# ultralytics/yolov3

Measured on AMD Instinct MI355X. Metric: images/sec (640x640) inference+NMS, higher is better.
Workload: dtype f16; 1 GPU; yolov3 inference 640x640 batch=32/GPU fp16 nc=80 + NMS(conf 0.001, iou 0.6, multi_label, max_det 300) [BASELINE configs[1]]; global_batch=32, parallelism=replicas x1 (no data-path collective)

## Files before the change

yolov3_amd/csrc/api.cpp:

```cpp
#include <atomic>
#include <mutex>
#include <stdarg.h>
#include <stdio.h>
#include <stdlib.h>
#include <string.h>

#include "../../include/yolov3_hip.h"
#include "y3_knobs.h"

static thread_local char g_err[512] = "";

void y3_set_error(const char* fmt, ...) {
    va_list ap;
    va_start(ap, fmt);
    vsnprintf(g_err, sizeof(g_err), fmt, ap);
    va_end(ap);
}

extern "C" const char* y3_last_error(void) { return g_err; }
extern "C" int y3_abi_version(void) { return Y3_ABI_VERSION; }

namespace {
struct Knob {
    const char* name;
    long long def;
};
const Knob kKnobs[] = {
    {"conv", 0}, {"conv_ahead", 3}, {"bn_nt_bytes", 64ll << 20},
    {"wgrad", 0}, {"wgrad_xcd", 2}, {"dgrad_quad", 1}, {"spp_direct", 0}, {"wgrad_strip", 1}, {"conv_strip", 1},
    {"conv_v10", 1}, {"v10_mp", 0}, {"v10_blocks", 0}, {"v10_half", 2}, {"v10_ksplit", 1}, {"v10_slices", 0},
    {"v10_group", 1}, {"tile_xcd", 1}, {"conv_1x1s", 1}, {"wgrad_patch", 1}, {"wgrad_blocks", 512}, {"nms_sort", 1},
    {"decode_tile", 1},
};
constexpr int kCount = (int)(sizeof(kKnobs) / sizeof(kKnobs[0]));
static_assert(kCount == Y3K_COUNT, "kKnobs and y3_knob_id (y3_common.h) list the same knobs in the same order");
std::atomic<long long> g_val[kCount];
std::once_flag g_once;

int knob_index(const char* key) {
    for (int i = 0; i < kCount; ++i)
        if (key && !strcmp(key, kKnobs[i].name)) return i;
    return -1;
}
void load_defaults() {
    for (int i = 0; i < kCount; ++i) g_val[i].store(kKnobs[i].def, std::memory_order_relaxed);
    const char* e = getenv("Y3_TUNE");
    if (!e) return;
    char buf[512];
    strncpy(buf, e, sizeof(buf) - 1);
    buf[sizeof(buf) - 1] = 0;
    for (char* tok = strtok(buf, ",;"); tok; tok = strtok(nullptr, ",;")) {
        char* eq = strchr(tok, '=');
        if (!eq) continue;
        *eq = 0;
        const int i = knob_index(tok);
        if (i >= 0) g_val[i].store(atoll(eq + 1), std::memory_order_relaxed);
        else fprintf(stderr, "libyolov3_hip: Y3_TUNE names an unknown knob '%s'\n", tok);
    }
}
}

long long y3_knob(int id) {
    std::call_once(g_once, load_defaults);
    return (id >= 0 && id < kCount) ? g_val[id].load(std::memory_order_relaxed) : 0;
}

extern "C" int y3_tune_set(const char* key, int64_t value) {
    std::call_once(g_once, load_defaults);
    const int i = knob_index(key);
    if (i < 0) {
        y3_set_error("y3_tune_set: unknown knob '%s'", key ? key : "(null)");
        return -1;
    }
    g_val[i].store((long long)value, std::memory_order_relaxed);
    return 0;
}

extern "C" int64_t y3_tune_get(const char* key) {
    std::call_once(g_once, load_defaults);
    const int i = knob_index(key);
    if (i < 0) {
        y3_set_error("y3_tune_get: unknown knob '%s'", key ? key : "(null)");
        return INT64_MIN;
    }
    return (int64_t)g_val[i].load(std::memory_order_relaxed);
}

extern "C" void y3_tune_reset(void) {
    std::call_once(g_once, load_defaults);
    load_defaults();
}
```

yolov3_amd/csrc/stem.hip:

```cpp
#include "../../include/yolov3_hip.h"
#include "y3_common.h"

#include <hip/hip_runtime.h>
#include <stdint.h>
#include <type_traits>
#include <utility>

namespace {

struct StemArgs {
    const void* x;
    const void* w;
    const float* bias;
    void* y;
    int N, Cin, H, W;
    int ypitch, Cout;
    int act;
    int tiles_w, tiles_h;
    float divisor;
    float* stats;
};

constexpr int TR = 8, TW = 64;
constexpr int PR = TR + 2;
// ... 117 lines not shown
        for (int i = 0; i < NI; ++i) {
            const int pl = i * PPI + rp;
            const frag ov = *(const frag*)(wl + pl * RB + ((ch ^ (pl & (CH - 1))) << 4));
            const int gcol = col0 + j0 + pl;
            if (grow < p.H && gcol < p.W && ch * 8 + 8 <= p.Cout) {
                if (want_stats) {
#pragma unroll
                    for (int q = 0; q < 8; ++q) { const float f = to_f32<T>(ov[q]); st0[q] += f; st1[q] += f * f; }
                }
                *(frag*)(yg + ((long long)(n * p.H + grow) * p.W + gcol) * p.ypitch + ch * 8) = ov;
            }
        }
        __builtin_amdgcn_fence(__ATOMIC_RELEASE, "wavefront");
        __builtin_amdgcn_wave_barrier();
    }
    if (want_stats) {
#pragma unroll
        for (int off = CH; off < 64; off <<= 1)
#pragma unroll
            for (int q = 0; q < 8; ++q) { st0[q] += __shfl_xor(st0[q], off, 64); st1[q] += __shfl_xor(st1[q], off, 64); }
        __syncthreads();
        float* red = (float*)patch;
        if (rp == 0) {
#pragma unroll
            for (int q = 0; q < 8; ++q) { red[(wv * CH + ch) * 16 + 2 * q] = st0[q]; red[(wv * CH + ch) * 16 + 2 * q + 1] = st1[q]; }
        }
        __syncthreads();
        if (tid < CH * 16 && (tid >> 4) * 8 + 8 <= p.Cout) {
            const float v = red[tid] + red[CH * 16 + tid] + red[2 * CH * 16 + tid] + red[3 * CH * 16 + tid];
            p.stats[(long long)blockIdx.x * p.Cout * 2 + tid] = v;
        }
    }
}

struct PairArgs {
    const void* x;
    const void* w0;
    const float* b0;
    const void* w1;
    const float* b1;
    void* y;
    int N, Cin, H, W, Ho, Wo, ypitch, act0, act1, kpad1;
    int tiles_w, tiles_h, n_tiles;
    int xcd;
    float divisor;
#ifdef Y3_TIMELINE
    unsigned long long* tl;
#endif
};
#ifdef Y3_TIMELINE
static unsigned long long* g_pair_tl = nullptr;
#define SP_T(i) do { asm volatile("s_waitcnt lgkmcnt(0)" ::: "memory"); const unsigned long long t_ = __builtin_amdgcn_s_memtime(); asm volatile("s_waitcnt lgkmcnt(0)" ::: "memory"); tsum[i] += t_ - tprev; tprev = t_; } while (0)
#else
#define SP_T(i) do { } while (0)
#endif
constexpr int QR = 4, QW = 32;
constexpr int R0 = 2 * QR + 1, C0 = 2 * QW + 1;
constexpr int XR = R0 + 2, XW = C0 + 3;
constexpr int L0E = C0 / 2 + 1, L0ROW = C0 * 64;

template <typename T, typename S>
__global__ __launch_bounds__(256, 2) void stem_pair_kernel(const PairArgs p) {
    typedef typename Mfma16<T>::frag frag;
    typedef T vec4 __attribute__((ext_vector_type(4)));
    typedef unsigned u32x4 __attribute__((ext_vector_type(4)));
    constexpr int PATCH_BYTES = XR * XW * 8, SLICE_BYTES = 4 * 32 * 64;
    constexpr int SCR = PATCH_BYTES > SLICE_BYTES ? PATCH_BYTES : SLICE_BYTES;
    __shared__ __attribute__((aligned(16))) unsigned char scratch[SCR];
    __shared__ __attribute__((aligned(16))) unsigned char l0buf[R0 * L0ROW];
    __shared__ __attribute__((aligned(16))) unsigned char cw0[32 * 48 * 2];
    __shared__ __attribute__((aligned(16))) float cb0[32], cb1[64];

    const int tid = threadIdx.x, lane = tid & 63;
    const int wv = __builtin_amdgcn_readfirstlane(tid >> 6);
    const int frow = lane & 31, fk = lane >> 5;
    const int wc = wv >> 1, wp = wv & 1;

    for (int i = tid; i < 32 * 48 * 2 / 16; i += 256) ((f32x4*)cw0)[i] = ((const f32x4*)p.w0)[i];
    if (tid < 8) ((f32x4*)cb0)[tid] = ((const f32x4*)p.b0)[tid];
    else if (tid < 24) ((f32x4*)cb1)[tid - 8] = ((const f32x4*)p.b1)[tid - 8];
    frag a1f[18];
#pragma unroll
    for (int t = 0; t < 18; ++t) a1f[t] = *(const frag*)((const T*)p.w1 + (long long)(wc * 32 + frow) * p.kpad1 + t * 16 + fk * 8);

    constexpr int NPX = (XR * XW + 255) / 256;
    int prc[NPX];
#pragma unroll
    for (int j = 0; j < NPX; ++j) {
        const int e = tid + j * 256;
        const int pr = e / XW;
        prc[j] = e < XR * XW ? (pr << 8) | (e - pr * XW) : -1;
    }
    constexpr int NT0 = (R0 * C0 + 31) / 32, NJ0 = (NT0 + 3) / 4;
    int l0rd[NJ0], l0wr[NJ0], l0rc[NJ0];
#pragma unroll
    for (int j = 0; j < NJ0; ++j) {
        int q = (wv + 4 * j) * 32 + frow;
        const bool live = q < R0 * C0;
        if (!live) q = R0 * C0 - 1;
        const int r = q / C0, c = q - r * C0, ci = c >> 1;
        l0rd[j] = (r * XW + c + 2 * fk) * 8;
        l0wr[j] = live ? r * L0ROW + ((c & 1) ? L0E * 64 : 0) + ci * 64 + ((fk ^ ((ci >> 2) & 3)) << 4) : -1;
        l0rc[j] = (r << 8) | c;
    }
    const int hw = p.H * p.W;

    T* __restrict__ yg = (T*)p.y;
    S raw[NPX][4];
    bool rin[NPX];
    auto fetch = [&](int tile) {
        int b = tile;
        const int tw = b % p.tiles_w; b /= p.tiles_w;
        const int th = b % p.tiles_h;
        const int n = b / p.tiles_h;
        const int gh0 = 2 * th * QR - 2, gw0 = 2 * tw * QW - 2;
        const S* __restrict__ xs = (const S*)p.x + (long long)n * p.Cin * hw;
#pragma unroll
        for (int j = 0; j < NPX; ++j) {
            const int gh = gh0 + (prc[j] >> 8), gw = gw0 + (prc[j] & 255);
            rin[j] = prc[j] >= 0 && (unsigned)gh < (unsigned)p.H && (unsigned)gw < (unsigned)p.W;
            if (rin[j]) {
                const unsigned o = (unsigned)(gh * p.W + gw);
#pragma unroll
                for (int c = 0; c < 4; ++c)
                    if (c < p.Cin) raw[j][c] = xs[o + (unsigned)(c * hw)];
            }
        }
    };
    const bool plain = std::is_same<S, T>::value && p.divisor == 1.0f;
    auto stash = [&]() {
#pragma unroll
        for (int j = 0; j < NPX; ++j) {
            const int e = tid + j * 256;
            if (e < XR * XW) {
                vec4 v = {(T)0.0f, (T)0.0f, (T)0.0f, (T)0.0f};
                if (rin[j]) {
                    bool done = false;
                    if constexpr (std::is_same<S, T>::value) {
                        if (plain) {
#pragma unroll
                            for (int c = 0; c < 4; ++c)
                                if (c < p.Cin) v[c] = raw[j][c];
                            done = true;
                        }
                    }
                    if (!done) {
#pragma unroll
                        for (int c = 0; c < 4; ++c)
                            if (c < p.Cin) v[c] = from_f32<T>(src_f32<S>(raw[j][c]) / p.divisor);
                    }
                }
                *(vec4*)(scratch + e * 8) = v;
            }
        }
    };
    const int first = p.xcd ? xcd_remap((int)blockIdx.x, (int)gridDim.x) : (int)blockIdx.x;
    if (first < p.n_tiles) fetch(first);
#ifdef Y3_TIMELINE
    unsigned long long tsum[8] = {0, 0, 0, 0, 0, 0, 0, 0};
    unsigned long long tprev = __builtin_amdgcn_s_memtime();
#endif
    for (int tile = first; tile < p.n_tiles; tile += gridDim.x) {
        int b = tile;
        const int tw = b % p.tiles_w; b /= p.tiles_w;
        const int th = b % p.tiles_h;
        const int n = b / p.tiles_h;
        const int oh0 = th * QR, ow0 = tw * QW;
        const int gh0 = 2 * oh0 - 1, gw0 = 2 * ow0 - 1;
        const bool border = gh0 < 0 || gw0 < 0 || gh0 + R0 > p.H || gw0 + C0 > p.W;

        stash();
        SP_T(0);
        __syncthreads();
        SP_T(1);

#pragma unroll
        for (int j = 0; j < NJ0; ++j) {
            if (wv + 4 * j >= NT0) break;
            f32x16 acc;
#pragma unroll
            for (int g = 0; g < 4; ++g)
#pragma unroll
                for (int e = 0; e < 4; ++e) acc[4 * g + e] = cb0[8 * g + 4 * fk + e];
#pragma unroll
            for (int kh = 0; kh < 3; ++kh) {
                const unsigned char* src = scratch + l0rd[j] + kh * (XW * 8);
                typedef unsigned long long u64x2 __attribute__((ext_vector_type(2)));
                u64x2 rw;
                rw[0] = *(const unsigned long long*)src;
                rw[1] = *(const unsigned long long*)(src + 8);
                acc = Mfma16<T>::run(*(const frag*)(cw0 + ((frow * 3 + kh) * 16 + fk * 8) * 2), __builtin_bit_cast(frag, rw), acc);
            }
            if (p.act0 == Y3_ACT_SILU) silu_vec<f32x16, 16>(acc);
            bool keep = l0wr[j] >= 0;
            bool inside = true;
            if (border) inside = (unsigned)(gh0 + (l0rc[j] >> 8)) < (unsigned)p.H && (unsigned)(gw0 + (l0rc[j] & 255)) < (unsigned)p.W;
#pragma unroll
            for (int gp = 0; gp < 2; ++gp) {
                u32x4 ov;
#pragma unroll
                for (int h = 0; h < 2; ++h) {
                    const unsigned a = pack2<T>(acc[8 * gp + 2 * h], acc[8 * gp + 2 * h + 1]);
                    const unsigned b = pack2<T>(acc[8 * gp + 4 + 2 * h], acc[8 * gp + 4 + 2 * h + 1]);
                    const auto sw = __builtin_amdgcn_permlane32_swap(a, b, false, false);
                    ov[h] = inside ? (unsigned)sw[0] : 0u;
                    ov[2 + h] = inside ? (unsigned)sw[1] : 0u;
                }
                if (keep) *(u32x4*)(l0buf + (l0wr[j] ^ (gp << 5))) = ov;
            }
        }
        SP_T(2);
        __syncthreads();
        SP_T(3);
        if (tile + (int)gridDim.x < p.n_tiles) fetch(tile + gridDim.x);

        f32x16 acc1[2];
#pragma unroll
        for (int b2 = 0; b2 < 2; ++b2)
#pragma unroll
            for (int g = 0; g < 4; ++g)
#pragma unroll
                for (int e = 0; e < 4; ++e) acc1[b2][4 * g + e] = cb1[wc * 32 + 8 * g + 4 * fk + e];
#pragma unroll
        for (int tap = 0; tap < 9; ++tap) {
            const int kh = tap / 3, kw = tap - 3 * (tap / 3);
#pragma unroll
            for (int ks = 0; ks < 2; ++ks)
#pragma unroll
                for (int b2 = 0; b2 < 2; ++b2) {
                    const int lr = 2 * wp + b2;
                    const int ci = frow + (kw >> 1);
                    const frag bf = *(const frag*)(l0buf + (2 * lr + kh) * L0ROW + ((kw & 1) ? L0E * 64 : 0) + ci * 64 + (((ks * 2 + fk) ^ ((ci >> 2) & 3)) << 4));
                    acc1[b2] = Mfma16<T>::run(a1f[tap * 2 + ks], bf, acc1[b2]);
                }
        }
        SP_T(4);
        unsigned char* wl = scratch + wv * (32 * 64);
        const int rp = lane >> 2, ch = lane & 3;
        if (p.act1 == Y3_ACT_SILU) {
            silu_vec<f32x16, 16>(acc1[0]);
            silu_vec<f32x16, 16>(acc1[1]);
        }
        const long long ybase = ((long long)(n * p.Ho + oh0 + 2 * wp) * p.Wo + ow0) * p.ypitch + wc * 32 + ch * 8;
#pragma unroll
        for (int b2 = 0; b2 < 2; ++b2) {
#pragma unroll
            for (int gp = 0; gp < 2; ++gp) {
                u32x4 ov;
#pragma unroll
                for (int h = 0; h < 2; ++h) {
                    const unsigned a = pack2<T>(acc1[b2][8 * gp + 2 * h], acc1[b2][8 * gp + 2 * h + 1]);
                    const unsigned b = pack2<T>(acc1[b2][8 * gp + 4 + 2 * h], acc1[b2][8 * gp + 4 + 2 * h + 1]);
                    const auto sw = __builtin_amdgcn_permlane32_swap(a, b, false, false);
                    ov[h] = (unsigned)sw[0];
                    ov[2 + h] = (unsigned)sw[1];
                }
                const int chunk = gp * 2 + fk;
                *(u32x4*)(wl + frow * 64 + ((chunk ^ (frow & 3)) << 4)) = ov;
            }
            __builtin_amdgcn_fence(__ATOMIC_RELEASE, "wavefront");
            __builtin_amdgcn_wave_barrier();
            __builtin_amdgcn_fence(__ATOMIC_ACQUIRE, "wavefront");
            const int oh = oh0 + 2 * wp + b2;
#pragma unroll
            for (int i = 0; i < 2; ++i) {
                const int pl = i * 16 + rp;
                const u32x4 ov = *(const u32x4*)(wl + pl * 64 + ((ch ^ (pl & 3)) << 4));
                if (oh < p.Ho && ow0 + pl < p.Wo) *(u32x4*)(yg + ybase + (long long)(b2 * p.Wo + pl) * p.ypitch) = ov;
            }
            __builtin_amdgcn_fence(__ATOMIC_RELEASE, "wavefront");
            __builtin_amdgcn_wave_barrier();
        }
        SP_T(5);
        __syncthreads();
        SP_T(6);
    }
#ifdef Y3_TIMELINE
    if (p.tl && blockIdx.x < 64 && lane == 0) {
#pragma unroll
        for (int i = 0; i < 8; ++i) p.tl[(blockIdx.x * 4 + wv) * 8 + i] = tsum[i];
    }
#endif
}

struct BneckArgs {
    const void* x;
    const void* w1;
    const float* b1;
    const void* w2;
    const float* b2;
    void* y;
    int N, H, W, xpitch, ypitch, act1, act2, add, kpad1, kpad2;
    int tiles_w, tiles_h, n_tiles;
    int xcd;
    unsigned x_bytes;
};
constexpr int BC = 32, RC = BC + 2;
constexpr int bneck_rows(int c) { return c == 64 ? 8 : 4; }
constexpr int L1PITCH = 40;

template <typename F, int... Is> Y3_DEV void sfor_impl(F&& f, std::integer_sequence<int, Is...>) { (f(std::integral_constant<int, Is>{}), ...); }
template <int N, typename F> Y3_DEV void sfor(F&& f) { sfor_impl(f, std::make_integer_sequence<int, N>{}); }

template <typename T, int C>
__global__ __launch_bounds__(C * 4, C == 64 ? 2 : 1) void bneck_pair_kernel(const BneckArgs p) {
    typedef typename Mfma16<T>::frag frag;
    typedef unsigned u32x4 __attribute__((ext_vector_type(4)));
    typedef __attribute__((address_space(3))) void* lds_ptr_t;
    constexpr int BR = bneck_rows(C), RW = BR / 2;
    constexpr int RR = BR + 2, RPX = RR * RC;
    constexpr int NT1 = (RPX + 31) / 32;
    constexpr int CM = C / 2;
    constexpr int FT = C / 32;
    constexpr int NWV = 2 * FT;
    constexpr int XB = C * 2, XCHK = XB / 16;
    constexpr int LB = CM * 2, LCHK = LB / 16;
    constexpr int K1S = C / 16, M1 = CM / 32;
    constexpr int KT = CM / 16;
    constexpr int K2S = 9 * KT;
    constexpr int XPIECES = (RPX * XCHK + 63) / 64;
    constexpr int XJ = (XPIECES + NWV - 1) / NWV;
    constexpr int NJ1 = (NT1 + NWV - 1) / NWV;
    constexpr int QSTEP = 32 * NWV;
    constexpr int XKS = XCHK == 8 ? 1 : 0;
    constexpr int LKS = LCHK == 4 ? 2 : 1;
    __shared__ __attribute__((aligned(16))) unsigned char xbuf[XPIECES * 1024];
    __shared__ __attribute__((aligned(16))) unsigned char l1buf[RR * L1PITCH * LB];
    __shared__ __attribute__((aligned(16))) unsigned char slices[NWV * 32 * 64];
    __shared__ __attribute__((aligned(16))) float cb1[CM], cb2[C];
    constexpr bool W1_LDS = C == 128;
    __shared__ __attribute__((aligned(16))) unsigned char cw1[W1_LDS ? CM * C * 2 : 16];

    const int tid = threadIdx.x, lane = tid & 63;
    const int wv = __builtin_amdgcn_readfirstlane(tid >> 6);
    const int frow = lane & 31, fk = lane >> 5;
    const int wc = wv >> 1, wp = wv & 1;

    if (tid < CM / 4) ((f32x4*)cb1)[tid] = ((const f32x4*)p.b1)[tid];
    else if (tid < CM / 4 + C / 4) ((f32x4*)cb2)[tid - CM / 4] = ((const f32x4*)p.b2)[tid - CM / 4];
    if constexpr (W1_LDS) {
        for (int i = tid; i < CM * XCHK; i += 64 * NWV) {
            const int r = i / XCHK, c = i % XCHK;
            *(u32x4*)(cw1 + r * XB + ((c ^ (r & 15)) << 4)) = *(const u32x4*)((const T*)p.w1 + (long long)r * p.kpad1 + c * 8);
        }
    }
    frag a2f[K2S];
#pragma unroll
    for (int t = 0; t < K2S; ++t) a2f[t] = *(const frag*)((const T*)p.w2 + (long long)(wc * 32 + frow) * p.kpad2 + t * 16 + fk * 8);

    const auto rs_x = __builtin_amdgcn_make_buffer_rsrc((void*)p.x, 0, (int)p.x_bytes, 0x00020000);
    const int c1q0 = 32 * wv + frow;
    const int c1r0 = c1q0 / RC, c1c0 = c1q0 - c1r0 * RC;
    const int c1rd0 = c1q0 * XB + ((fk ^ ((c1q0 >> XKS) & (XCHK - 1))) << 4);
    int c2rd[3];
#pragma unroll
    for (int kw = 0; kw < 3; ++kw) c2rd[kw] = (frow + kw) * LB + ((fk ^ (((frow + kw) >> LKS) & (LCHK - 1))) << 4);

    T* __restrict__ yg = (T*)p.y;
    auto fetch = [&](int tile) {
        int b = tile;
        const int tw = b % p.tiles_w; b /= p.tiles_w;
        const int th = b % p.tiles_h;
        const int n = b / p.tiles_h;
        const int gh0 = th * BR - 1, gw0 = tw * BC - 1;
        int lane_f = lane;
        asm volatile("" : "+v"(lane_f));
        const int xq0 = (64 / XCHK) * wv + lane_f / XCHK;
        const unsigned xsrc = (unsigned)(((lane_f % XCHK) ^ ((xq0 >> XKS) & (XCHK - 1))) * 16);
        int r = 0, c = xq0;
#pragma unroll
        for (int j = 0; j < XJ; ++j) {
            if (wv + NWV * j >= XPIECES) break;
            const int gh = gh0 + r, gw = gw0 + c;
            const bool ok = xq0 + 32 * j < RPX && (unsigned)gh < (unsigned)p.H && (unsigned)gw < (unsigned)p.W;
            const unsigned off = ok ? (unsigned)(((n * p.H + gh) * p.W + gw) * p.xpitch) * 2u + xsrc : 0xffffffffu;
            const unsigned ldsa = __builtin_amdgcn_readfirstlane((unsigned)(uintptr_t)(lds_ptr_t)xbuf + (unsigned)((wv + NWV * j) * 1024));
            asm volatile("s_mov_b32 m0, %0\n\ts_nop 0\n\tbuffer_load_dwordx4 %1, %2, 0 offen lds" : : "s"(ldsa), "v"(off), "s"(rs_x) : "memory");
            c += 32;
            if (c >= RC) { c -= RC; r += 1; }
        }
    };
    const int first = p.xcd ? xcd_remap((int)blockIdx.x, (int)gridDim.x) : (int)blockIdx.x;
    if (first < p.n_tiles) fetch(first);
    for (int tile = first; tile < p.n_tiles; tile += gridDim.x) {
        int b = tile;
        const int tw = b % p.tiles_w; b /= p.tiles_w;
        const int th = b % p.tiles_h;
        const int n = b / p.tiles_h;
        const int oh0 = th * BR, ow0 = tw * BC;
        const int gh0 = oh0 - 1, gw0 = ow0 - 1;
        const bool border = gh0 < 0 || gw0 < 0 || gh0 + RR > p.H || gw0 + RC > p.W;

        frag a1g[W1_LDS ? 1 : K1S * M1];
        if constexpr (!W1_LDS) {
#pragma unroll
            for (int ks = 0; ks < K1S; ++ks)
#pragma unroll
                for (int m = 0; m < M1; ++m) a1g[ks * M1 + m] = *(const frag*)((const T*)p.w1 + (long long)(m * 32 + frow) * p.kpad1 + ks * 16 + fk * 8);
        }
        __builtin_amdgcn_s_waitcnt(0x0F70);
        __syncthreads();

        {
            f32x16 acc[NJ1][M1];
#pragma unroll
            for (int j = 0; j < NJ1; ++j)
#pragma unroll
                for (int m = 0; m < M1; ++m)
#pragma unroll
                    for (int g = 0; g < 4; ++g)
#pragma unroll
                        for (int e = 0; e < 4; ++e) acc[j][m][4 * g + e] = cb1[m * 32 + 8 * g + 4 * fk + e];
#pragma unroll
            for (int ks = 0; ks < K1S; ++ks) {
                frag af[M1];
#pragma unroll
                for (int m = 0; m < M1; ++m) {
                    if constexpr (W1_LDS) af[m] = *(const frag*)(cw1 + (m * 32 + frow) * XB + (((2 * ks + fk) ^ (frow & 15)) << 4));
                    else af[m] = a1g[ks * M1 + m];
                }
#pragma unroll
                for (int j = 0; j < NJ1; ++j) {
                    if (wv + NWV * j >= NT1) break;
                    const frag bf = *(const frag*)(xbuf + ((c1rd0 + j * (QSTEP * XB)) ^ (ks << 5)));
#pragma unroll
                    for (int m = 0; m < M1; ++m) acc[j][m] = Mfma16<T>::run(af[m], bf, acc[j][m]);
                }
            }
            int r1 = c1r0, c1 = c1c0;
#pragma unroll
            for (int j = 0; j < NJ1; ++j) {
                if (wv + NWV * j >= NT1) break;
                const bool live = c1q0 + QSTEP * j < RPX;
                bool inside = true;
                if (border) inside = (unsigned)(gh0 + r1) < (unsigned)p.H && (unsigned)(gw0 + c1) < (unsigned)p.W;
                const int wr = (r1 * L1PITCH + c1) * LB + ((fk ^ ((c1 >> LKS) & (LCHK - 1)) ^ ((r1 & 1) * (LCHK / 2))) << 4);
#pragma unroll
                for (int m = 0; m < M1; ++m) {
                    if (p.act1 == Y3_ACT_SILU) silu_vec<f32x16, 16>(acc[j][m]);
#pragma unroll
                    for (int gp = 0; gp < 2; ++gp) {
                        u32x4 ov;
#pragma unroll
                        for (int h = 0; h < 2; ++h) {
                            const auto sw = __builtin_amdgcn_permlane32_swap(pack2<T>(acc[j][m][8 * gp + 2 * h], acc[j][m][8 * gp + 2 * h + 1]),
                                                                             pack2<T>(acc[j][m][8 * gp + 4 + 2 * h], acc[j][m][8 * gp + 4 + 2 * h + 1]), false, false);
                            ov[h] = inside ? (unsigned)sw[0] : 0u;
                            ov[2 + h] = inside ? (unsigned)sw[1] : 0u;
                        }
                        if (live) *(u32x4*)(l1buf + (wr ^ ((m * 4 + gp * 2) << 4))) = ov;
                    }
                    __builtin_amdgcn_sched_barrier(0);
                }
                c1 += QSTEP % RC;
                r1 += QSTEP / RC;
                if (c1 >= RC) { c1 -= RC; r1 += 1; }
            }
        }
        u32x4 xres[2 * RW];
        if (p.add) {
            int lane_r = lane;
            asm volatile("" : "+v"(lane_r));
            const int rp_r = lane_r >> 2, lc = wc * 4 + (lane_r & 3);
#pragma unroll
            for (int b2 = 0; b2 < RW; ++b2)
#pragma unroll
                for (int i = 0; i < 2; ++i) {
                    const int q = (RW * wp + b2 + 1) * RC + (i * 16 + rp_r + 1);
                    xres[b2 * 2 + i] = *(const u32x4*)(xbuf + q * XB + ((lc ^ ((q >> XKS) & (XCHK - 1))) << 4));
                }
        }
        __syncthreads();
        {
            int nt = tile + (int)gridDim.x;
            asm volatile("" : "+s"(nt));
            if (nt < p.n_tiles) fetch(nt);
        }
        f32x16 acc2[RW];
#pragma unroll
        for (int b2 = 0; b2 < RW; ++b2)
#pragma unroll
            for (int g = 0; g < 4; ++g)
#pragma unroll
                for (int e = 0; e < 4; ++e) acc2[b2][4 * g + e] = cb2[wc * 32 + 8 * g + 4 * fk + e];
        const unsigned char* l1w = l1buf + (RW * wp) * (L1PITCH * LB);
        auto rd = [&](auto step_c, frag (&bf)[RW]) {
            constexpr int tap = decltype(step_c)::value / KT, ks = decltype(step_c)::value % KT, kh = tap / 3, kw = tap - 3 * (tap / 3);
#pragma unroll
            for (int b2 = 0; b2 < RW; ++b2) {
                const int rr = b2 + kh;
                bf[b2] = *(const frag*)(l1w + rr * (L1PITCH * LB) + (c2rd[kw] ^ (((2 * ks) ^ ((rr & 1) * (LCHK / 2))) << 4)));
            }
        };
        auto mm = [&](auto step_c, const frag (&bf)[RW]) {
#pragma unroll
            for (int b2 = 0; b2 < RW; ++b2) acc2[b2] = Mfma16<T>::run(a2f[decltype(step_c)::value], bf[b2], acc2[b2]);
        };
        frag bA[RW], bB[RW];
        rd(std::integral_constant<int, 0>{}, bA);
        __builtin_amdgcn_sched_barrier(0);
        sfor<K2S / 2 - 1>([&](auto i_c) {
            constexpr int s0 = 2 * decltype(i_c)::value;
            rd(std::integral_constant<int, s0 + 1>{}, bB);
            mm(std::integral_constant<int, s0>{}, bA);
            __builtin_amdgcn_sched_barrier(0);
            rd(std::integral_constant<int, s0 + 2>{}, bA);
            mm(std::integral_constant<int, s0 + 1>{}, bB);
            __builtin_amdgcn_sched_barrier(0);
        });
        rd(std::integral_constant<int, K2S - 1>{}, bB);
        mm(std::integral_constant<int, K2S - 2>{}, bA);
        __builtin_amdgcn_sched_barrier(0);
        mm(std::integral_constant<int, K2S - 1>{}, bB);
        __builtin_amdgcn_sched_barrier(0);
        int lane_o = lane;
        asm volatile("" : "+v"(lane_o));
        const int rp = lane_o >> 2, ch = lane_o & 3;
        unsigned char* wl = slices + wv * (32 * 64);
        if (p.act2 == Y3_ACT_SILU) {
#pragma unroll
            for (int b2 = 0; b2 < RW; ++b2) {
                silu_vec<f32x16, 16>(acc2[b2]);
                __builtin_amdgcn_sched_barrier(0);
            }
        }
        const long long ybase = ((long long)(n * p.H + oh0 + RW * wp) * p.W + ow0) * p.ypitch + wc * 32 + ch * 8;
#pragma unroll
        for (int b2 = 0; b2 < RW; ++b2) {
#pragma unroll
            for (int gp = 0; gp < 2; ++gp) {
                u32x4 ov;
#pragma unroll
                for (int h = 0; h < 2; ++h) {
                    const auto sw = __builtin_amdgcn_permlane32_swap(pack2<T>(acc2[b2][8 * gp + 2 * h], acc2[b2][8 * gp + 2 * h + 1]),
                                                                     pack2<T>(acc2[b2][8 * gp + 4 + 2 * h], acc2[b2][8 * gp + 4 + 2 * h + 1]), false, false);
                    ov[h] = (unsigned)sw[0];
                    ov[2 + h] = (unsigned)sw[1];
                }
                const int chunk = gp * 2 + fk;
                *(u32x4*)(wl + frow * 64 + ((chunk ^ (frow & 3)) << 4)) = ov;
            }
            __builtin_amdgcn_fence(__ATOMIC_RELEASE, "wavefront");
            __builtin_amdgcn_wave_barrier();
            __builtin_amdgcn_fence(__ATOMIC_ACQUIRE, "wavefront");
            const int orow = RW * wp + b2;
#pragma unroll
            for (int i = 0; i < 2; ++i) {
                const int pl = i * 16 + rp;
                frag ov = *(const frag*)(wl + pl * 64 + ((ch ^ (pl & 3)) << 4));
                if (p.add) {
                    const frag xr = __builtin_bit_cast(frag, xres[b2 * 2 + i]);
                    u32x4 sum;
#pragma unroll
                    for (int e = 0; e < 8; e += 2) sum[e >> 1] = pack2<T>(to_f32<T>(ov[e]) + to_f32<T>(xr[e]), to_f32<T>(ov[e + 1]) + to_f32<T>(xr[e + 1]));
                    ov = __builtin_bit_cast(frag, sum);
                }
                if (oh0 + orow < p.H && ow0 + pl < p.W) *(frag*)(yg + ybase + (long long)(b2 * p.W + pl) * p.ypitch) = ov;
            }
            __builtin_amdgcn_fence(__ATOMIC_RELEASE, "wavefront");
            __builtin_amdgcn_wave_barrier();
        }
        __syncthreads();
    }
}

template <typename T, typename S> int launch_stem(const StemArgs& a, hipStream_t st) {
    const dim3 grid((unsigned)((long long)a.tiles_w * a.tiles_h * a.N));
    if (a.Cout <= 32)
        hipLaunchKernelGGL((stem_conv_kernel<T, S, 1>), grid, dim3(256), 0, st, a);
    else
        hipLaunchKernelGGL((stem_conv_kernel<T, S, 2>), grid, dim3(256), 0, st, a);
    Y3_CHECK_LAUNCH();
    return 0;
}

template <typename T> int dispatch_src(const StemArgs& a, int sdt, hipStream_t st) {
    switch (sdt) {
        case Y3_F16: return launch_stem<T, f16_t>(a, st);
        case Y3_BF16: return launch_stem<T, bf16_t>(a, st);
        case Y3_F32: return launch_stem<T, float>(a, st);
        case Y3_U8: return launch_stem<T, unsigned char>(a, st);
    }
    Y3_FAIL("y3_stem_conv_fwd: bad source dtype %d", sdt);
}

}

static int stem_conv_impl(const void* x_nchw, int32_t src_dtype, int32_t n, int32_t cin, int32_t h, int32_t w, float divisor, const void* packed, const float* bias,
                          int32_t dtype, int32_t act, const y3_tensor* y, float* stat_rows, int64_t capacity_rows, int64_t* n_rows, void* stream, const char* who) {
    if (!x_nchw || !packed || !y || !y->data) Y3_FAIL("%s: null argument", who);
    if (cin < 1 || cin > 4) Y3_FAIL("%s: %d input channels (1..4 supported)", who, cin);
    if (y->n != n || y->h != h || y->w != w) Y3_FAIL("%s: output must be (%d,%d,%d,*) for a stride-1 pad-1 3x3", who, n, h, w);
    if ((y->c % 8) || y->c > 64 || (y->pitch % 8) || ((uintptr_t)y->data & 15) || ((uintptr_t)packed & 15)) Y3_FAIL("%s: 8..64 filters (multiple of 8), 16-byte aligned views", who);
    if (!(divisor > 0.0f)) Y3_FAIL("%s: divisor must be positive", who);
    if ((long long)n * h * w > 0x7fffffffLL) Y3_FAIL("%s: too many pixels", who);
    StemArgs a;
    a.x = x_nchw; a.w = packed; a.bias = bias; a.y = y->data;
    a.N = n; a.Cin = cin; a.H = h; a.W = w; a.ypitch = y->pitch; a.Cout = y->c; a.act = act;
    a.tiles_w = (w + TW - 1) / TW; a.tiles_h = (h + TR - 1) / TR;
    a.divisor = divisor;
    a.stats = stat_rows;
    const long long rows = (long long)a.tiles_w * a.tiles_h * n;
    if (stat_rows) {
        if (rows > capacity_rows) Y3_FAIL("%s: %lld statistics rows, capacity %lld", who, rows, (long long)capacity_rows);
        if (n_rows) *n_rows = rows;
    }
    hipStream_t st = (hipStream_t)stream;
    switch (dtype) {
        case Y3_F16: return dispatch_src<f16_t>(a, src_dtype, st);
        case Y3_BF16: return dispatch_src<bf16_t>(a, src_dtype, st);
    }
    Y3_FAIL("%s: f16/bf16 compute only", who);
}

extern "C" int y3_stem_conv_fwd(const void* x_nchw, int32_t src_dtype, int32_t n, int32_t cin, int32_t h, int32_t w, float divisor, const void* packed,
                                const float* bias, int32_t dtype, int32_t act, const y3_tensor* y, void* stream) {
    return stem_conv_impl(x_nchw, src_dtype, n, cin, h, w, divisor, packed, bias, dtype, act, y, nullptr, 0, nullptr, stream, "y3_stem_conv_fwd");
}

extern "C" int64_t y3_stem_conv_stats_rows(int32_t n, int32_t h, int32_t w) { return (int64_t)((w + TW - 1) / TW) * ((h + TR - 1) / TR) * n; }

extern "C" int y3_stem_conv_fwd_stats(const void* x_nchw, int32_t src_dtype, int32_t n, int32_t cin, int32_t h, int32_t w, float divisor, const void* packed,
                                      const float* bias, int32_t dtype, int32_t act, const y3_tensor* y, float* stat_rows, int64_t capacity_rows, int64_t* n_rows,
                                      void* stream) {
    if (!stat_rows || !n_rows) Y3_FAIL("y3_stem_conv_fwd_stats: null statistics buffer");
    return stem_conv_impl(x_nchw, src_dtype, n, cin, h, w, divisor, packed, bias, dtype, act, y, stat_rows, capacity_rows, n_rows, stream, "y3_stem_conv_fwd_stats");
}

namespace {
template <typename T> int dispatch_pair(const PairArgs& a, int sdt, long long tiles, hipStream_t st) {
    const int cap = 2 * y3_cu_count();
    const int blocks = tiles < cap ? (int)tiles : cap;
    switch (sdt) {
        case Y3_F16: hipLaunchKernelGGL((stem_pair_kernel<T, f16_t>), dim3((unsigned)blocks), dim3(256), 0, st, a); break;
        case Y3_BF16: hipLaunchKernelGGL((stem_pair_kernel<T, bf16_t>), dim3((unsigned)blocks), dim3(256), 0, st, a); break;
        case Y3_F32: hipLaunchKernelGGL((stem_pair_kernel<T, float>), dim3((unsigned)blocks), dim3(256), 0, st, a); break;
        case Y3_U8: hipLaunchKernelGGL((stem_pair_kernel<T, unsigned char>), dim3((unsigned)blocks), dim3(256), 0, st, a); break;
        default: Y3_FAIL("y3_stem_pair_fwd: bad source dtype %d", sdt);
    }
    Y3_CHECK_LAUNCH();
    return 0;
}
}

#ifdef Y3_TIMELINE
extern "C" void y3_debug_pair_timeline(void* buf) { g_pair_tl = (unsigned long long*)buf; }
#endif

extern "C" int y3_stem_pair_fwd(const void* x_nchw, int32_t src_dtype, int32_t n, int32_t cin, int32_t h, int32_t w, float divisor, const void* packed0, const float* bias0,
                                int32_t act0, const void* packed1, const float* bias1, int32_t act1, int32_t dtype, const y3_tensor* y, void* stream) {
    if (!x_nchw || !packed0 || !bias0 || !packed1 || !bias1 || !y || !y->data) Y3_FAIL("y3_stem_pair_fwd: null argument");
    if (cin < 1 || cin > 4) Y3_FAIL("y3_stem_pair_fwd: %d input channels (1..4 supported)", cin);
    const int Ho = (h - 1) / 2 + 1, Wo = (w - 1) / 2 + 1;
    if (y->n != n || y->h != Ho || y->w != Wo || y->c != 64) Y3_FAIL("y3_stem_pair_fwd: output must be (%d,%d,%d,64)", n, Ho, Wo);
    if ((y->pitch % 8) || ((uintptr_t)y->data & 15) || ((uintptr_t)packed0 & 15) || ((uintptr_t)packed1 & 15) || ((uintptr_t)bias0 & 15) || ((uintptr_t)bias1 & 15))
        Y3_FAIL("y3_stem_pair_fwd: 16-byte aligned views");
    if (!(divisor > 0.0f)) Y3_FAIL("y3_stem_pair_fwd: divisor must be positive");
    if ((long long)n * h * w > 0x7fffffffLL) Y3_FAIL("y3_stem_pair_fwd: too many pixels");
    PairArgs a;
    a.x = x_nchw; a.w0 = packed0; a.b0 = bias0; a.w1 = packed1; a.b1 = bias1; a.y = y->data;
    a.N = n; a.Cin = cin; a.H = h; a.W = w; a.Ho = Ho; a.Wo = Wo; a.ypitch = y->pitch; a.act0 = act0; a.act1 = act1;
    a.kpad1 = y3_filter_kpad(32, 3);
    a.tiles_w = (Wo + QW - 1) / QW; a.tiles_h = (Ho + QR - 1) / QR;
    const long long tiles = (long long)a.tiles_w * a.tiles_h * n;
    if (tiles > 0x7fffffffLL) Y3_FAIL("y3_stem_pair_fwd: too many tiles");
    a.n_tiles = (int)tiles;
    a.xcd = y3_knob(Y3K_TILE_XCD) != 0;
    a.divisor = divisor;
#ifdef Y3_TIMELINE
    a.tl = g_pair_tl;
#endif
    hipStream_t st = (hipStream_t)stream;
    switch (dtype) {
        case Y3_F16: return dispatch_pair<f16_t>(a, src_dtype, tiles, st);
        case Y3_BF16: return dispatch_pair<bf16_t>(a, src_dtype, tiles, st);
    }
    Y3_FAIL("y3_stem_pair_fwd: f16/bf16 compute only");
}

extern "C" int y3_bneck_pair_fwd(const y3_tensor* x, const void* packed1, const float* bias1, int32_t act1, const void* packed2, const float* bias2, int32_t act2,
                                 int32_t add_residual, int32_t dtype, const y3_tensor* y, void* stream) {
    if (!x || !x->data || !packed1 || !bias1 || !packed2 || !bias2 || !y || !y->data) Y3_FAIL("y3_bneck_pair_fwd: null argument");
    const int c = x->c;
    if ((c != 64 && c != 128) || y->c != c) Y3_FAIL("y3_bneck_pair_fwd: Bottleneck(64, 64) or Bottleneck(128, 128) (cv1 C -> C/2 1x1, cv2 C/2 -> C 3x3), got %d -> %d channels", x->c, y->c);
    if (y->n != x->n || y->h != x->h || y->w != x->w) Y3_FAIL("y3_bneck_pair_fwd: output shape");
    if ((x->pitch % 8) || (y->pitch % 8) || ((uintptr_t)x->data & 15) || ((uintptr_t)y->data & 15) || ((uintptr_t)packed1 & 15) || ((uintptr_t)packed2 & 15) ||
        ((uintptr_t)bias1 & 15) || ((uintptr_t)bias2 & 15))
        Y3_FAIL("y3_bneck_pair_fwd: 16-byte aligned views");
    if (x->data == y->data) Y3_FAIL("y3_bneck_pair_fwd: in-place operation is not supported (tiles read their neighbours' input)");
    BneckArgs a;
    a.x = x->data; a.w1 = packed1; a.b1 = bias1; a.w2 = packed2; a.b2 = bias2; a.y = y->data;
    a.N = x->n; a.H = x->h; a.W = x->w; a.xpitch = x->pitch; a.ypitch = y->pitch; a.act1 = act1; a.act2 = act2; a.add = add_residual ? 1 : 0;
    a.kpad1 = y3_filter_kpad(c, 1); a.kpad2 = y3_filter_kpad(c / 2, 3);
    a.tiles_w = (x->w + BC - 1) / BC; a.tiles_h = (x->h + bneck_rows(c) - 1) / bneck_rows(c);
    const long long tiles = (long long)a.tiles_w * a.tiles_h * x->n;
    if (tiles > 0x7fffffffLL || (long long)x->n * x->h * x->w > 0x7fffffffLL) Y3_FAIL("y3_bneck_pair_fwd: too many pixels");
    a.n_tiles = (int)tiles;
    a.xcd = y3_knob(Y3K_TILE_XCD) != 0;
    const long long xb = (((long long)x->n * x->h * x->w - 1) * x->pitch + x->c) * 2;
    if (xb >= 0x7fffffffLL) Y3_FAIL("y3_bneck_pair_fwd: input beyond the 2 GiB reach of a buffer descriptor (split the batch)");
    a.x_bytes = (unsigned)xb;
    const int cap = (c == 64 ? 2 : 1) * y3_cu_count();
    const int blocks = tiles < cap ? (int)tiles : cap;
    hipStream_t st = (hipStream_t)stream;
    if (dtype != Y3_F16 && dtype != Y3_BF16) Y3_FAIL("y3_bneck_pair_fwd: f16/bf16 only");
    if (c == 64) {
        if (dtype == Y3_F16) hipLaunchKernelGGL((bneck_pair_kernel<f16_t, 64>), dim3((unsigned)blocks), dim3(256), 0, st, a);
        else hipLaunchKernelGGL((bneck_pair_kernel<bf16_t, 64>), dim3((unsigned)blocks), dim3(256), 0, st, a);
    } else {
        if (dtype == Y3_F16) hipLaunchKernelGGL((bneck_pair_kernel<f16_t, 128>), dim3((unsigned)blocks), dim3(512), 0, st, a);
        else hipLaunchKernelGGL((bneck_pair_kernel<bf16_t, 128>), dim3((unsigned)blocks), dim3(512), 0, st, a);
    }
    Y3_CHECK_LAUNCH();
    return 0;
}
```

yolov3_amd/csrc/y3_knobs.h:

```cpp
#pragma once
enum y3_knob_id {
    Y3K_CONV = 0,
    Y3K_CONV_AHEAD,
    Y3K_BN_NT_BYTES,
    Y3K_WGRAD,
    Y3K_WGRAD_XCD,
    Y3K_DGRAD_QUAD,
    Y3K_SPP_DIRECT,
    Y3K_WGRAD_STRIP,
    Y3K_CONV_STRIP,
    Y3K_CONV_V10,
    Y3K_V10_MP,
    Y3K_V10_BLOCKS,
    Y3K_V10_HALF,
    Y3K_V10_KSPLIT,
    Y3K_V10_SLICES,
    Y3K_V10_GROUP,
    Y3K_TILE_XCD,
    Y3K_CONV_1X1S,
    Y3K_WGRAD_PATCH,
    Y3K_WGRAD_BLOCKS,
    Y3K_NMS_SORT,
    Y3K_DECODE_TILE,
    Y3K_COUNT
};
long long y3_knob(int id);
```

Before: 5235 images/sec.

## Pipeline bottleneck-pair epilogue into next row's MFMAs and hoist w1 fragment loads

Adds a PIPE variant of the fused bottleneck-pair kernel, selected by a new pair_pipe knob that is on by default. The variant interleaves each output row's SiLU, permlane packing, LDS transpose and global store into the MFMA stream of the following row, using a three-deep B-fragment rotation. It also loads the 1x1 weight fragments once per block instead of once per tile. The aim is to hide epilogue latency and cut repeated global weight loads, at the cost of more register pressure and a fragile, hand-placed schedule.

```diff
diff --git a/yolov3_amd/csrc/api.cpp b/yolov3_amd/csrc/api.cpp
--- a/yolov3_amd/csrc/api.cpp
+++ b/yolov3_amd/csrc/api.cpp
@@ -30,7 +30,7 @@
     {"wgrad", 0}, {"wgrad_xcd", 2}, {"dgrad_quad", 1}, {"spp_direct", 0}, {"wgrad_strip", 1}, {"conv_strip", 1},
     {"conv_v10", 1}, {"v10_mp", 0}, {"v10_blocks", 0}, {"v10_half", 2}, {"v10_ksplit", 1}, {"v10_slices", 0},
     {"v10_group", 1}, {"tile_xcd", 1}, {"conv_1x1s", 1}, {"wgrad_patch", 1}, {"wgrad_blocks", 512}, {"nms_sort", 1},
-    {"decode_tile", 1},
+    {"decode_tile", 1}, {"pair_pipe", 1},
 };
 constexpr int kCount = (int)(sizeof(kKnobs) / sizeof(kKnobs[0]));
 static_assert(kCount == Y3K_COUNT, "kKnobs and y3_knob_id (y3_common.h) list the same knobs in the same order");
diff --git a/yolov3_amd/csrc/stem.hip b/yolov3_amd/csrc/stem.hip
--- a/yolov3_amd/csrc/stem.hip
+++ b/yolov3_amd/csrc/stem.hip
@@ -443,7 +443,7 @@
 template <typename F, int... Is> Y3_DEV void sfor_impl(F&& f, std::integer_sequence<int, Is...>) { (f(std::integral_constant<int, Is>{}), ...); }
 template <int N, typename F> Y3_DEV void sfor(F&& f) { sfor_impl(f, std::make_integer_sequence<int, N>{}); }
 
-template <typename T, int C>
+template <typename T, int C, int PIPE>
 __global__ __launch_bounds__(C * 4, C == 64 ? 2 : 1) void bneck_pair_kernel(const BneckArgs p) {
     typedef typename Mfma16<T>::frag frag;
     typedef unsigned u32x4 __attribute__((ext_vector_type(4)));
@@ -490,9 +490,6 @@
     for (int t = 0; t < K2S; ++t) a2f[t] = *(const frag*)((const T*)p.w2 + (long long)(wc * 32 + frow) * p.kpad2 + t * 16 + fk * 8);
 
     const auto rs_x = __builtin_amdgcn_make_buffer_rsrc((void*)p.x, 0, (int)p.x_bytes, 0x00020000);
-    const int c1q0 = 32 * wv + frow;
-    const int c1r0 = c1q0 / RC, c1c0 = c1q0 - c1r0 * RC;
-    const int c1rd0 = c1q0 * XB + ((fk ^ ((c1q0 >> XKS) & (XCHK - 1))) << 4);
     int c2rd[3];
 #pragma unroll
     for (int kw = 0; kw < 3; ++kw) c2rd[kw] = (frow + kw) * LB + ((fk ^ (((frow + kw) >> LKS) & (LCHK - 1))) << 4);
@@ -523,6 +520,19 @@
     };
     const int first = p.xcd ? xcd_remap((int)blockIdx.x, (int)gridDim.x) : (int)blockIdx.x;
     if (first < p.n_tiles) fetch(first);
+    frag a1g[W1_LDS ? 1 : K1S * M1];
+    auto load_a1g = [&]() {
+        if constexpr (!W1_LDS) {
+#pragma unroll
+            for (int ks = 0; ks < K1S; ++ks)
+#pragma unroll
+                for (int m = 0; m < M1; ++m) a1g[ks * M1 + m] = *(const frag*)((const T*)p.w1 + (long long)(m * 32 + frow) * p.kpad1 + ks * 16 + fk * 8);
+        }
+    };
+    if constexpr (PIPE) {
+        load_a1g();
+        __builtin_amdgcn_s_waitcnt(0x0F70);
+    }
     for (int tile = first; tile < p.n_tiles; tile += gridDim.x) {
         int b = tile;
         const int tw = b % p.tiles_w; b /= p.tiles_w;
@@ -532,14 +542,13 @@
         const int gh0 = oh0 - 1, gw0 = ow0 - 1;
         const bool border = gh0 < 0 || gw0 < 0 || gh0 + RR > p.H || gw0 + RC > p.W;
 
-        frag a1g[W1_LDS ? 1 : K1S * M1];
-        if constexpr (!W1_LDS) {
-#pragma unroll
-            for (int ks = 0; ks < K1S; ++ks)
-#pragma unroll
-                for (int m = 0; m < M1; ++m) a1g[ks * M1 + m] = *(const frag*)((const T*)p.w1 + (long long)(m * 32 + frow) * p.kpad1 + ks * 16 + fk * 8);
-        }
-        __builtin_amdgcn_s_waitcnt(0x0F70);
+        int lane_c = lane;
+        if constexpr (PIPE) asm volatile("" : "+v"(lane_c));
+        const int c1q0 = 32 * wv + (lane_c & 31);
+        const int c1r0 = c1q0 / RC, c1c0 = c1q0 - c1r0 * RC;
+        const int c1rd0 = c1q0 * XB + (((lane_c >> 5) ^ ((c1q0 >> XKS) & (XCHK - 1))) << 4);
+        if constexpr (!PIPE) load_a1g();
+        if constexpr (!PIPE) __builtin_amdgcn_s_waitcnt(0x0F70);
         __syncthreads();
 
         {
@@ -625,81 +634,169 @@
 #pragma unroll
                 for (int e = 0; e < 4; ++e) acc2[b2][4 * g + e] = cb2[wc * 32 + 8 * g + 4 * fk + e];
         const unsigned char* l1w = l1buf + (RW * wp) * (L1PITCH * LB);
-        auto rd = [&](auto step_c, frag (&bf)[RW]) {
-            constexpr int tap = decltype(step_c)::value / KT, ks = decltype(step_c)::value % KT, kh = tap / 3, kw = tap - 3 * (tap / 3);
+        if constexpr (!PIPE) {
+            auto rd = [&](auto step_c, frag (&bf)[RW]) {
+                constexpr int tap = decltype(step_c)::value / KT, ks = decltype(step_c)::value % KT, kh = tap / 3, kw = tap - 3 * (tap / 3);
+#pragma unroll
+                for (int b2 = 0; b2 < RW; ++b2) {
+                    const int rr = b2 + kh;
+                    bf[b2] = *(const frag*)(l1w + rr * (L1PITCH * LB) + (c2rd[kw] ^ (((2 * ks) ^ ((rr & 1) * (LCHK / 2))) << 4)));
+                }
+            };
+            auto mm = [&](auto step_c, const frag (&bf)[RW]) {
+#pragma unroll
+                for (int b2 = 0; b2 < RW; ++b2) acc2[b2] = Mfma16<T>::run(a2f[decltype(step_c)::value], bf[b2], acc2[b2]);
+            };
+            frag bA[RW], bB[RW];
+            rd(std::integral_constant<int, 0>{}, bA);
+            __builtin_amdgcn_sched_barrier(0);
+            sfor<K2S / 2 - 1>([&](auto i_c) {
+                constexpr int s0 = 2 * decltype(i_c)::value;
+                rd(std::integral_constant<int, s0 + 1>{}, bB);
+                mm(std::integral_constant<int, s0>{}, bA);
+                __builtin_amdgcn_sched_barrier(0);
+                rd(std::integral_constant<int, s0 + 2>{}, bA);
+                mm(std::integral_constant<int, s0 + 1>{}, bB);
+                __builtin_amdgcn_sched_barrier(0);
+            });
+            rd(std::integral_constant<int, K2S - 1>{}, bB);
+            mm(std::integral_constant<int, K2S - 2>{}, bA);
+            __builtin_amdgcn_sched_barrier(0);
+            mm(std::integral_constant<int, K2S - 1>{}, bB);
+            __builtin_amdgcn_sched_barrier(0);
+            int lane_o = lane;
+            asm volatile("" : "+v"(lane_o));
+            const int rp = lane_o >> 2, ch = lane_o & 3;
+            unsigned char* wl = slices + wv * (32 * 64);
+            if (p.act2 == Y3_ACT_SILU) {
+#pragma unroll
+                for (int b2 = 0; b2 < RW; ++b2) {
+                    silu_vec<f32x16, 16>(acc2[b2]);
+                    __builtin_amdgcn_sched_barrier(0);
+                }
+            }
+            const long long ybase = ((long long)(n * p.H + oh0 + RW * wp) * p.W + ow0) * p.ypitch + wc * 32 + ch * 8;
 #pragma unroll
             for (int b2 = 0; b2 < RW; ++b2) {
-                const int rr = b2 + kh;
-                bf[b2] = *(const frag*)(l1w + rr * (L1PITCH * LB) + (c2rd[kw] ^ (((2 * ks) ^ ((rr & 1) * (LCHK / 2))) << 4)));
-            }
-        };
-        auto mm = [&](auto step_c, const frag (&bf)[RW]) {
-#pragma unroll
-            for (int b2 = 0; b2 < RW; ++b2) acc2[b2] = Mfma16<T>::run(a2f[decltype(step_c)::value], bf[b2], acc2[b2]);
-        };
-        frag bA[RW], bB[RW];
-        rd(std::integral_constant<int, 0>{}, bA);
-        __builtin_amdgcn_sched_barrier(0);
-        sfor<K2S / 2 - 1>([&](auto i_c) {
-            constexpr int s0 = 2 * decltype(i_c)::value;
-            rd(std::integral_constant<int, s0 + 1>{}, bB);
-            mm(std::integral_constant<int, s0>{}, bA);
-            __builtin_amdgcn_sched_barrier(0);
-            rd(std::integral_constant<int, s0 + 2>{}, bA);
-            mm(std::integral_constant<int, s0 + 1>{}, bB);
-            __builtin_amdgcn_sched_barrier(0);
-        });
-        rd(std::integral_constant<int, K2S - 1>{}, bB);
-        mm(std::integral_constant<int, K2S - 2>{}, bA);
-        __builtin_amdgcn_sched_barrier(0);
-        mm(std::integral_constant<int, K2S - 1>{}, bB);
-        __builtin_amdgcn_sched_barrier(0);
-        int lane_o = lane;
-        asm volatile("" : "+v"(lane_o));
-        const int rp = lane_o >> 2, ch = lane_o & 3;
-        unsigned char* wl = slices + wv * (32 * 64);
-        if (p.act2 == Y3_ACT_SILU) {
-#pragma unroll
-            for (int b2 = 0; b2 < RW; ++b2) {
-                silu_vec<f32x16, 16>(acc2[b2]);
+#pragma unroll
+                for (int gp = 0; gp < 2; ++gp) {
+                    u32x4 ov;
+#pragma unroll
+                    for (int h = 0; h < 2; ++h) {
+                        const auto sw = __builtin_amdgcn_permlane32_swap(pack2<T>(acc2[b2][8 * gp + 2 * h], acc2[b2][8 * gp + 2 * h + 1]),
+                                                                         pack2<T>(acc2[b2][8 * gp + 4 + 2 * h], acc2[b2][8 * gp + 4 + 2 * h + 1]), false, false);
+                        ov[h] = (unsigned)sw[0];
+                        ov[2 + h] = (unsigned)sw[1];
+                    }
+                    const int chunk = gp * 2 + fk;
+                    *(u32x4*)(wl + frow * 64 + ((chunk ^ (frow & 3)) << 4)) = ov;
+                }
+                __builtin_amdgcn_fence(__ATOMIC_RELEASE, "wavefront");
+                __builtin_amdgcn_wave_barrier();
+                __builtin_amdgcn_fence(__ATOMIC_ACQUIRE, "wavefront");
+                const int orow = RW * wp + b2;
+#pragma unroll
+                for (int i = 0; i < 2; ++i) {
+                    const int pl = i * 16 + rp;
+                    frag ov = *(const frag*)(wl + pl * 64 + ((ch ^ (pl & 3)) << 4));
+                    if (p.add) {
+                        const frag xr = __builtin_bit_cast(frag, xres[b2 * 2 + i]);
+                        u32x4 sum;
+#pragma unroll
+                        for (int e = 0; e < 8; e += 2) sum[e >> 1] = pack2<T>(to_f32<T>(ov[e]) + to_f32<T>(xr[e]), to_f32<T>(ov[e + 1]) + to_f32<T>(xr[e + 1]));
+                        ov = __builtin_bit_cast(frag, sum);
+                    }
+                    if (oh0 + orow < p.H && ow0 + pl < p.W) *(frag*)(yg + ybase + (long long)(b2 * p.W + pl) * p.ypitch) = ov;
+                }
+                __builtin_amdgcn_fence(__ATOMIC_RELEASE, "wavefront");
+                __builtin_amdgcn_wave_barrier();
+            }
+        } else {
+            constexpr int QS = K2S >= 36 ? 5 : 2;
+            constexpr int SW0 = QS + (QS > 2 ? 2 : 1), SW1 = 3 * QS + (QS > 2 ? 2 : 1);
+            constexpr int SRD = 3 * QS + (QS > 2 ? 5 : 3), SST = SRD + 3, SEND = SRD + 7;
+            static_assert(SW0 > QS && SW1 > 3 * QS && SRD > SW1 && SEND < K2S, "the epilogue of a row fits into the MFMAs of the next");
+            const long long ybase = ((long long)(n * p.H + oh0 + RW * wp) * p.W + ow0) * p.ypitch + wc * 32;
+            unsigned char* wl = slices + wv * (32 * 64);
+            frag so[2];
+            auto epi = [&](auto row_c, auto s_c, auto silu_c) {
+                constexpr int b2 = decltype(row_c)::value, s = decltype(s_c)::value;
+                if constexpr (decltype(silu_c)::value && s % QS == 0 && s / QS < 4) {
+                    constexpr int q = 4 * (s / QS);
+                    f32x4 v = {acc2[b2][q], acc2[b2][q + 1], acc2[b2][q + 2], acc2[b2][q + 3]};
+                    silu_vec<f32x4, 4>(v);
+#pragma unroll
+                    for (int e = 0; e < 4; ++e) acc2[b2][q + e] = v[e];
+                }
+                if constexpr (s == SW0 || s == SW1) {
+                    constexpr int gp = s == SW1 ? 1 : 0;
+                    u32x4 ov;
+#pragma unroll
+                    for (int h = 0; h < 2; ++h) {
+                        const auto sw = __builtin_amdgcn_permlane32_swap(pack2<T>(acc2[b2][8 * gp + 2 * h], acc2[b2][8 * gp + 2 * h + 1]),
+                                                                         pack2<T>(acc2[b2][8 * gp + 4 + 2 * h], acc2[b2][8 * gp + 4 + 2 * h + 1]), false, false);
+                        ov[h] = (unsigned)sw[0];
+                        ov[2 + h] = (unsigned)sw[1];
+                    }
+                    const int chunk = gp * 2 + fk;
+                    *(u32x4*)(wl + frow * 64 + ((chunk ^ (frow & 3)) << 4)) = ov;
+                }
+                if constexpr (s == SRD) {
+                    __builtin_amdgcn_fence(__ATOMIC_RELEASE, "wavefront");
+                    __builtin_amdgcn_wave_barrier();
+                    __builtin_amdgcn_fence(__ATOMIC_ACQUIRE, "wavefront");
+                    int lane_o = lane;
+                    asm volatile("" : "+v"(lane_o));
+                    const int rp = lane_o >> 2, ch = lane_o & 3;
+#pragma unroll
+                    for (int i = 0; i < 2; ++i) {
+                        const int pl = i * 16 + rp;
+                        so[i] = *(const frag*)(wl + pl * 64 + ((ch ^ (pl & 3)) << 4));
+                    }
+                }
+                if constexpr (s == SST || s == SST + 2) {
+                    constexpr int i = (s - SST) / 2;
+                    int lane_o = lane;
+                    asm volatile("" : "+v"(lane_o));
+                    const int pl = i * 16 + (lane_o >> 2);
+                    frag ov = so[i];
+                    if (p.add) {
+                        const frag xr = __builtin_bit_cast(frag, xres[b2 * 2 + i]);
+                        u32x4 sum;
+#pragma unroll
+                        for (int e = 0; e < 8; e += 2) sum[e >> 1] = pack2<T>(to_f32<T>(ov[e]) + to_f32<T>(xr[e]), to_f32<T>(ov[e + 1]) + to_f32<T>(xr[e + 1]));
+                        ov = __builtin_bit_cast(frag, sum);
+                    }
+                    if (oh0 + RW * wp + b2 < p.H && ow0 + pl < p.W) *(frag*)(yg + ybase + (lane_o & 3) * 8 + (long long)(b2 * p.W + pl) * p.ypitch) = ov;
+                }
+                if constexpr (s == SEND) {
+                    __builtin_amdgcn_fence(__ATOMIC_RELEASE, "wavefront");
+                    __builtin_amdgcn_wave_barrier();
+                }
+            };
+            auto rd1 = [&](auto g_c, frag& bf) {
+                constexpr int b2 = decltype(g_c)::value / K2S, st = decltype(g_c)::value % K2S;
+                constexpr int tap = st / KT, ks = st % KT, kh = tap / 3, kw = tap - 3 * (tap / 3);
+                constexpr int rr = b2 + kh;
+                bf = *(const frag*)(l1w + rr * (L1PITCH * LB) + (c2rd[kw] ^ (((2 * ks) ^ ((rr & 1) * (LCHK / 2))) << 4)));
+            };
+            auto rows = [&](auto silu_c) {
+                frag fb[3];
+                rd1(std::integral_constant<int, 0>{}, fb[0]);
+                rd1(std::integral_constant<int, 1>{}, fb[1]);
                 __builtin_amdgcn_sched_barrier(0);
-            }
-        }
-        const long long ybase = ((long long)(n * p.H + oh0 + RW * wp) * p.W + ow0) * p.ypitch + wc * 32 + ch * 8;
-#pragma unroll
-        for (int b2 = 0; b2 < RW; ++b2) {
-#pragma unroll
-            for (int gp = 0; gp < 2; ++gp) {
-                u32x4 ov;
-#pragma unroll
-                for (int h = 0; h < 2; ++h) {
-                    const auto sw = __builtin_amdgcn_permlane32_swap(pack2<T>(acc2[b2][8 * gp + 2 * h], acc2[b2][8 * gp + 2 * h + 1]),
-                                                                     pack2<T>(acc2[b2][8 * gp + 4 + 2 * h], acc2[b2][8 * gp + 4 + 2 * h + 1]), false, false);
-                    ov[h] = (unsigned)sw[0];
-                    ov[2 + h] = (unsigned)sw[1];
-                }
-                const int chunk = gp * 2 + fk;
-                *(u32x4*)(wl + frow * 64 + ((chunk ^ (frow & 3)) << 4)) = ov;
-            }
-            __builtin_amdgcn_fence(__ATOMIC_RELEASE, "wavefront");
-            __builtin_amdgcn_wave_barrier();
-            __builtin_amdgcn_fence(__ATOMIC_ACQUIRE, "wavefront");
-            const int orow = RW * wp + b2;
-#pragma unroll
-            for (int i = 0; i < 2; ++i) {
-                const int pl = i * 16 + rp;
-                frag ov = *(const frag*)(wl + pl * 64 + ((ch ^ (pl & 3)) << 4));
-                if (p.add) {
-                    const frag xr = __builtin_bit_cast(frag, xres[b2 * 2 + i]);
-                    u32x4 sum;
-#pragma unroll
-                    for (int e = 0; e < 8; e += 2) sum[e >> 1] = pack2<T>(to_f32<T>(ov[e]) + to_f32<T>(xr[e]), to_f32<T>(ov[e + 1]) + to_f32<T>(xr[e + 1]));
-                    ov = __builtin_bit_cast(frag, sum);
-                }
-                if (oh0 + orow < p.H && ow0 + pl < p.W) *(frag*)(yg + ybase + (long long)(b2 * p.W + pl) * p.ypitch) = ov;
-            }
-            __builtin_amdgcn_fence(__ATOMIC_RELEASE, "wavefront");
-            __builtin_amdgcn_wave_barrier();
+                sfor<RW * K2S>([&](auto g_c) {
+                    constexpr int g = decltype(g_c)::value, b2 = g / K2S, s = g % K2S;
+                    if constexpr (g + 2 < RW * K2S) rd1(std::integral_constant<int, g + 2>{}, fb[(g + 2) % 3]);
+                    acc2[b2] = Mfma16<T>::run(a2f[s], fb[g % 3], acc2[b2]);
+                    if constexpr (b2 > 0) epi(std::integral_constant<int, b2 - 1>{}, std::integral_constant<int, s>{}, silu_c);
+                    __builtin_amdgcn_sched_barrier(0);
+                });
+                __builtin_amdgcn_s_waitcnt(0x0F70);
+                sfor<K2S>([&](auto s_c) { epi(std::integral_constant<int, RW - 1>{}, s_c, silu_c); });
+            };
+            if (p.act2 == Y3_ACT_SILU) rows(std::true_type{});
+            else rows(std::false_type{});
         }
         __syncthreads();
     }
@@ -778,6 +875,20 @@
         case Y3_F32: hipLaunchKernelGGL((stem_pair_kernel<T, float>), dim3((unsigned)blocks), dim3(256), 0, st, a); break;
         case Y3_U8: hipLaunchKernelGGL((stem_pair_kernel<T, unsigned char>), dim3((unsigned)blocks), dim3(256), 0, st, a); break;
         default: Y3_FAIL("y3_stem_pair_fwd: bad source dtype %d", sdt);
+    }
+    Y3_CHECK_LAUNCH();
+    return 0;
+}
+}
+
+namespace {
+template <int PIPE> int launch_bneck(const BneckArgs& a, int c, int dtype, int blocks, hipStream_t st) {
+    if (c == 64) {
+        if (dtype == Y3_F16) hipLaunchKernelGGL((bneck_pair_kernel<f16_t, 64, PIPE>), dim3((unsigned)blocks), dim3(256), 0, st, a);
+        else hipLaunchKernelGGL((bneck_pair_kernel<bf16_t, 64, PIPE>), dim3((unsigned)blocks), dim3(256), 0, st, a);
+    } else {
+        if (dtype == Y3_F16) hipLaunchKernelGGL((bneck_pair_kernel<f16_t, 128, PIPE>), dim3((unsigned)blocks), dim3(512), 0, st, a);
+        else hipLaunchKernelGGL((bneck_pair_kernel<bf16_t, 128, PIPE>), dim3((unsigned)blocks), dim3(512), 0, st, a);
     }
     Y3_CHECK_LAUNCH();
     return 0;
@@ -845,13 +956,6 @@
     const int blocks = tiles < cap ? (int)tiles : cap;
     hipStream_t st = (hipStream_t)stream;
     if (dtype != Y3_F16 && dtype != Y3_BF16) Y3_FAIL("y3_bneck_pair_fwd: f16/bf16 only");
-    if (c == 64) {
-        if (dtype == Y3_F16) hipLaunchKernelGGL((bneck_pair_kernel<f16_t, 64>), dim3((unsigned)blocks), dim3(256), 0, st, a);
-        else hipLaunchKernelGGL((bneck_pair_kernel<bf16_t, 64>), dim3((unsigned)blocks), dim3(256), 0, st, a);
-    } else {
-        if (dtype == Y3_F16) hipLaunchKernelGGL((bneck_pair_kernel<f16_t, 128>), dim3((unsigned)blocks), dim3(512), 0, st, a);
-        else hipLaunchKernelGGL((bneck_pair_kernel<bf16_t, 128>), dim3((unsigned)blocks), dim3(512), 0, st, a);
-    }
-    Y3_CHECK_LAUNCH();
-    return 0;
-}
+    if (y3_knob(Y3K_PAIR_PIPE) != 0) return launch_bneck<1>(a, c, dtype, blocks, st);
+    return launch_bneck<0>(a, c, dtype, blocks, st);
+}
diff --git a/yolov3_amd/csrc/y3_knobs.h b/yolov3_amd/csrc/y3_knobs.h
--- a/yolov3_amd/csrc/y3_knobs.h
+++ b/yolov3_amd/csrc/y3_knobs.h
@@ -22,6 +22,7 @@
     Y3K_WGRAD_BLOCKS,
     Y3K_NMS_SORT,
     Y3K_DECODE_TILE,
+    Y3K_PAIR_PIPE,
     Y3K_COUNT
 };
 long long y3_knob(int id);
```

After: 5282 images/sec (median of 6 runs). About the same (+0.9%).
